# TimZaman/dotaclient

Measured on NVIDIA H100. Metric: optimizer_steps_per_sec, higher is better.
Workload: dtype f32

## Files before the change

### dotaclient_b200/csrc/gemm_tf32x3.cu

```cuda
#include "dc_common.cuh"
#include "unit_basic.cuh"

namespace {

constexpr int BM = 128, BN = 128, BK = 32;
constexpr int kStages = 2;
constexpr int kTileBytes = BM * BK * 4;
constexpr int kStageBytes = 4 * kTileBytes;
constexpr int kProducerThreads = 128;
constexpr int kProducerGroups = kStages;
constexpr int kConsumerWarp0 = 4 * kProducerGroups;
constexpr int kConsumerThreads = 256;
constexpr int kThreads = kConsumerWarp0 * 32 + kConsumerThreads;
constexpr int kLdS = BN + 8;
constexpr int kDIn = kUnitFeatures;
constexpr size_t kOffStaging = (size_t)kStages * kStageBytes;
constexpr size_t kOffBars = kOffStaging + (size_t)BM * kLdS * 4;
constexpr size_t kSmemBytes = kOffBars + 128 + 1024 ;

#define DC_ACC8(b) "+f"(d[b]), "+f"(d[b + 1]), "+f"(d[b + 2]), "+f"(d[b + 3]), "+f"(d[b + 4]), "+f"(d[b + 5]), "+f"(d[b + 6]), "+f"(d[b + 7])
__device__ __forceinline__ void wgmma_m64n128k8(float (&d)[64], uint64_t desc_a, uint64_t desc_b) {
    asm volatile(
        "{\n\t.reg .pred p;\n\tsetp.ne.b32 p, %66, 0;\n\t"
        "wgmma.mma_async.sync.aligned.m64n128k8.f32.tf32.tf32 "
// ... 130 lines not shown
            const float4 a4 = dl != nullptr ? __ldg(reinterpret_cast<const float4 *>(att + nn * 128 + k0) + c) : zero4;
            const float gl = dl != nullptr ? __ldg(dl + nn * ld_dl) : 0.f;
            raw.v[i] = ok ? make_float4(fmaf(gl, a4.x, d.x), fmaf(gl, a4.y, d.y), fmaf(gl, a4.z, d.z), fmaf(gl, a4.w, d.w)) : zero4;
        }
    } else {
        constexpr int kTileToks = (BM - BM % NU) / NU;
#pragma unroll
        for (int k = 0; k < DembRaw<NU>::kP; ++k) {
            const int p = t + kProducerThreads * k;
            const int c = p & 7, tokl = NU == 16 ? p >> 4 : p >> 3;
            const int u0 = NU == 16 ? ((p >> 3) & 1) * 8 : 0;
            const bool active = tokl < kTileToks;
            const int n = tok0 + tokl;
            raw.ok[k] = active && n < n_tok;
            const size_t nn = (size_t)min(n, n_tok - 1);
            float4 d = (active && dx != nullptr) ? __ldg(reinterpret_cast<const float4 *>(dx + nn * ld_dx + k0) + c) : zero4;
            const float4 d2 = (active && dx2 != nullptr) ? __ldg(reinterpret_cast<const float4 *>(dx2 + nn * ld_dx + k0) + c) : zero4;
            if constexpr (NU == 16) {
                raw.d2[k] = d2;
            } else {
                d.x += d2.x; d.y += d2.y; d.z += d2.z; d.w += d2.w;
            }
            raw.d[k] = d;
            raw.am[k] = (active && dx != nullptr) ? __ldg(reinterpret_cast<const uint32_t *>(argmax + nn * 128 + k0) + c) : 0u;
            raw.a[k] = (active && dl != nullptr) ? __ldg(reinterpret_cast<const float4 *>(att + nn * 128 + k0) + c) : zero4;
#pragma unroll
            for (int j = 0; j < DembRaw<NU>::kU; ++j) raw.g[k][j] = (active && dl != nullptr) ? __ldg(dl + nn * ld_dl + u0 + j) : 0.f;
        }
    }
}

__device__ __forceinline__ void store_hi_lo(unsigned char *dst_hi, unsigned char *dst_lo, int off, float4 o) {
    float4 hi, lo;
    hi.x = dc_tf32_rna(o.x); hi.y = dc_tf32_rna(o.y); hi.z = dc_tf32_rna(o.z); hi.w = dc_tf32_rna(o.w);
    lo.x = o.x - hi.x; lo.y = o.y - hi.y; lo.z = o.z - hi.z; lo.w = o.w - hi.w;
    *reinterpret_cast<float4 *>(dst_hi + off) = hi;
    *reinterpret_cast<float4 *>(dst_lo + off) = lo;
}

template <int NU>
__device__ __forceinline__ void demb_store(const DembRaw<NU> &raw, unsigned char *dst_hi, unsigned char *dst_lo, int t) {
    if constexpr (NU == 1) {
        tile_store_k(raw.v, dst_hi, dst_lo, t);
    } else {
        constexpr int kTileRows = BM - BM % NU, kTileToks = kTileRows / NU;
        const float4 zero4 = make_float4(0.f, 0.f, 0.f, 0.f);
#pragma unroll
        for (int k = 0; k < DembRaw<NU>::kP; ++k) {
            const int p = t + kProducerThreads * k;
            const int c = p & 7, tokl = NU == 16 ? p >> 4 : p >> 3;
            const int u0 = NU == 16 ? ((p >> 3) & 1) * 8 : 0;
            if (tokl < kTileToks) {
                float4 d = raw.d[k];
                if constexpr (NU == 16) { d.x += raw.d2[k].x; d.y += raw.d2[k].y; d.z += raw.d2[k].z; d.w += raw.d2[k].w; }
                const float4 a = raw.a[k];
                const uint32_t am = raw.am[k];
#pragma unroll
                for (int j = 0; j < DembRaw<NU>::kU; ++j) {
                    const int u = u0 + j, r = tokl * NU + u;
                    const float gl = raw.g[k][j];
                    float4 o;
                    o.x = fmaf(gl, a.x, (int)(am & 0xffu) == u ? d.x : 0.f);
                    o.y = fmaf(gl, a.y, (int)((am >> 8) & 0xffu) == u ? d.y : 0.f);
                    o.z = fmaf(gl, a.z, (int)((am >> 16) & 0xffu) == u ? d.z : 0.f);
                    o.w = fmaf(gl, a.w, (int)(am >> 24) == u ? d.w : 0.f);
                    store_hi_lo(dst_hi, dst_lo, r * 128 + ((c ^ (r & 7)) << 4), raw.ok[k] ? o : zero4);
                }
            }
        }
        if constexpr (kTileRows < BM) {
            if (t < (BM - kTileRows) * 8) {
                const int r = kTileRows + (t >> 3), c = t & 7;
                store_hi_lo(dst_hi, dst_lo, r * 128 + ((c ^ (r & 7)) << 4), zero4);
            }
        }
    }
}

__device__ __forceinline__ void store_row_k(const float (&v)[32], unsigned char *dst_hi, unsigned char *dst_lo, int row) {
#pragma unroll
    for (int c = 0; c < 8; ++c) {
        const int off = row * 128 + ((c ^ (row & 7)) << 4);
        float4 hi, lo;
        hi.x = dc_tf32_rna(v[4 * c]); hi.y = dc_tf32_rna(v[4 * c + 1]); hi.z = dc_tf32_rna(v[4 * c + 2]); hi.w = dc_tf32_rna(v[4 * c + 3]);
        lo.x = v[4 * c] - hi.x; lo.y = v[4 * c + 1] - hi.y; lo.z = v[4 * c + 2] - hi.z; lo.w = v[4 * c + 3] - hi.w;
        *reinterpret_cast<float4 *>(dst_hi + off) = hi;
        *reinterpret_cast<float4 *>(dst_lo + off) = lo;
    }
}

__global__ void __launch_bounds__(kThreads, 1) gemm_tf32x3_kernel(const float *__restrict__ A, int lda,
                                                                  const float *__restrict__ B, int ldb,
                                                                  const float *__restrict__ bias, float *__restrict__ C,
                                                                  int ldc, int M, int N, int K, int relu, int ksplit,
                                                                  long long c_split_stride) {
    constexpr int kTileRows = BM;
    extern __shared__ unsigned char smem_raw[];
    unsigned char *tiles = smem_base(smem_raw);
    float *S = reinterpret_cast<float *>(tiles + kOffStaging);
    uint64_t *full = reinterpret_cast<uint64_t *>(tiles + kOffBars), *empty = full + kStages;

    const int warp = threadIdx.x >> 5, lane = threadIdx.x & 31;
    const int m_blocks = (M + kTileRows - 1) / kTileRows, n_blocks = (N + BN - 1) / BN, k_chunks = K / BK / ksplit;
    const int tiles_mn = m_blocks * n_blocks, tiles_total = tiles_mn * ksplit;
    init_ring(full);

    if (warp < kConsumerWarp0) {
        const int t = threadIdx.x & (kProducerThreads - 1), g = warp >> 2;
        uint32_t c = 0;
        for (int tile = blockIdx.x; tile < tiles_total; tile += gridDim.x) {
            const int tmn = tile % tiles_mn, kc0 = (tile / tiles_mn) * k_chunks;
            const int m0 = (tmn / n_blocks) * kTileRows, n0 = (tmn % n_blocks) * BN;
            for (int kc = 0; kc < k_chunks; ++kc, ++c) {
                if ((int)(c % kProducerGroups) != g) continue;
                float4 va[8], vb[8];
                tile_load_k(A, lda, m0, M, (kc0 + kc) * BK, t, va);
                tile_load_k(B, ldb, n0, N, (kc0 + kc) * BK, t, vb);
                produce(full, empty, c, lane, [&](int s) {
                    unsigned char *st = tiles + (size_t)s * kStageBytes;
                    tile_store_k(va, st, st + kTileBytes, t);
                    tile_store_k(vb, st + 2 * kTileBytes, st + 3 * kTileBytes, t);
                });
            }
        }
    } else {
        const int ct = threadIdx.x - kConsumerWarp0 * 32, wg = ct >> 7, cw = ct >> 5;
        float d[64];
        uint32_t c = 0;
        for (int tile = blockIdx.x; tile < tiles_total; tile += gridDim.x) {
            const int tmn = tile % tiles_mn, sp = tile / tiles_mn;
            const int m0 = (tmn / n_blocks) * kTileRows, n0 = (tmn % n_blocks) * BN;
            consume(d, tiles, full, empty, c, k_chunks, wg, lane);
            consumer_sync();
            stage_acc(d, S, ct);
            consumer_sync();
            const bool lane_in = n0 + 4 * lane < N;
            const bool has_bias = bias != nullptr && sp == 0 && lane_in;
            const float4 b4 = has_bias ? __ldg(reinterpret_cast<const float4 *>(bias + n0) + lane) : make_float4(0.f, 0.f, 0.f, 0.f);
            float *cbase = C + (size_t)sp * (size_t)c_split_stride + n0 + 4 * lane;
            for (int r = cw; lane_in && r < BM && m0 + r < M; r += kConsumerThreads / 32) {
                float4 v = *reinterpret_cast<const float4 *>(S + r * kLdS + 4 * lane);
                if (has_bias) { v.x += b4.x; v.y += b4.y; v.z += b4.z; v.w += b4.w; }
                if (relu) { v.x = fmaxf(v.x, 0.f); v.y = fmaxf(v.y, 0.f); v.z = fmaxf(v.z, 0.f); v.w = fmaxf(v.w, 0.f); }
                *reinterpret_cast<float4 *>(cbase + (size_t)(m0 + r) * ldc) = v;
            }
        }
    }
}

constexpr int kWsRows = 64;
constexpr int kWsStages = 8;
constexpr int kWsChunkBytes = kWsRows * BK * 4;
constexpr int kWsThreads = kConsumerThreads + 128;
constexpr int kWsLdS = 40;
constexpr size_t kWsOffRing = (size_t)4 * 2 * kTileBytes;
constexpr size_t kWsOffStaging = kWsOffRing + (size_t)kWsStages * kWsChunkBytes;
constexpr size_t kWsOffBars = kWsOffStaging + (size_t)(kConsumerThreads / 32) * 16 * kWsLdS * 4;
constexpr size_t kWsSmemBytes = kWsOffBars + 2 * kWsStages * 8 + 1024 ;
constexpr size_t kWsOffUnits = kWsOffBars + 2 * kWsStages * 8;
constexpr size_t kWsGenSmemBytes = kWsOffUnits + (size_t)4 * kWsRows * kDIn * 4 + 1024 ;
static_assert(kWsSmemBytes <= 227 * 1024 && kWsGenSmemBytes <= 227 * 1024, "weight-stationary GEMM exceeds the shared-memory opt-in");
static_assert(kWsOffUnits % 16 == 0, "unit rows are staged with 16-byte stores");

struct GenA {
    const float *units, *w_b, *b_b;
    float *basic_out;
    uint32_t *mask_out;
};

__device__ __forceinline__ void cp_async16(uint32_t dst, const void *src, uint32_t src_bytes) {
    asm volatile("cp.async.cg.shared.global [%0], [%1], 16, %2;" ::"r"(dst), "l"(src), "r"(src_bytes) : "memory");
}
__device__ __forceinline__ void cp_async_arrive(uint64_t *bar) {
    asm volatile("cp.async.mbarrier.arrive.noinc.shared::cta.b64 [%0];" ::"r"(dc_smem_u32(bar)) : "memory");
}

#define DC_ACC8(b) "+f"(d[b]), "+f"(d[b + 1]), "+f"(d[b + 2]), "+f"(d[b + 3]), "+f"(d[b + 4]), "+f"(d[b + 5]), "+f"(d[b + 6]), "+f"(d[b + 7])
__device__ __forceinline__ void wgmma_m64n128k8_rs(float (&d)[64], uint32_t a0, uint32_t a1, uint32_t a2, uint32_t a3, uint64_t desc_b) {
    asm volatile(
        "{\n\t.reg .pred p;\n\tsetp.ne.b32 p, %69, 0;\n\t"
        "wgmma.mma_async.sync.aligned.m64n128k8.f32.tf32.tf32 "
        "{%0, %1, %2, %3, %4, %5, %6, %7, %8, %9, %10, %11, %12, %13, %14, %15, "
        "%16, %17, %18, %19, %20, %21, %22, %23, %24, %25, %26, %27, %28, %29, %30, %31, "
        "%32, %33, %34, %35, %36, %37, %38, %39, %40, %41, %42, %43, %44, %45, %46, %47, "
        "%48, %49, %50, %51, %52, %53, %54, %55, %56, %57, %58, %59, %60, %61, %62, %63}, "
        "{%64, %65, %66, %67}, %68, p, 1, 1;\n\t}\n"
        : DC_ACC8(0), DC_ACC8(8), DC_ACC8(16), DC_ACC8(24), DC_ACC8(32), DC_ACC8(40), DC_ACC8(48), DC_ACC8(56)
        : "r"(a0), "r"(a1), "r"(a2), "r"(a3), "l"(desc_b), "r"(1));
}
#undef DC_ACC8

__device__ __forceinline__ void ws_fetch(float (&v)[16], const float *chunk, int rlo, int rhi, bool hi_ok, int q) {
#pragma unroll
    for (int ks = 0; ks < BK / 8; ++ks) {
#pragma unroll
        for (int h = 0; h < 2; ++h) {
            const int j = 2 * ks + h;
            v[4 * ks + 2 * h] = chunk[rlo * BK + ((j ^ (rlo & 7)) << 2) + q];
            v[4 * ks + 2 * h + 1] = hi_ok ? chunk[rhi * BK + ((j ^ (rhi & 7)) << 2) + q] : 0.f;
        }
    }
}

template <int NU, bool kGenA>
__global__ void __launch_bounds__(kWsThreads, 1) gemm_ws_kernel(const float *__restrict__ A, int lda,
                                                                const float *__restrict__ B, int ldb,
                                                                const float *__restrict__ bias, float *__restrict__ C,
                                                                int ldc, int M, int N, int K, int relu,
                                                                float *__restrict__ C_copy, uint8_t *__restrict__ argmax, GenA gen) {
    constexpr int kWarpRows = NU == 5 ? 15 : 16;
    constexpr int kTileRows = 4 * kWarpRows;
    extern __shared__ unsigned char smem_raw[];
    unsigned char *sm = smem_base(smem_raw);
    unsigned char *ring = sm + kWsOffRing;
    uint64_t *full = reinterpret_cast<uint64_t *>(sm + kWsOffBars), *empty = full + kWsStages;

    const int warp = threadIdx.x >> 5, lane = threadIdx.x & 31;
    const int n_blocks = (N + BN - 1) / BN, m_blocks = (M + kTileRows - 1) / kTileRows, k_chunks = K / BK;
    const int n0 = (blockIdx.x % n_blocks) * BN, mb0 = blockIdx.x / n_blocks, mstride = gridDim.x / n_blocks;
    if (threadIdx.x == 0) {
        for (int s = 0; s < kWsStages; ++s) { dc_mbar_init(&full[s], kGenA ? 1 : 128); dc_mbar_init(&empty[s], 4); }
        asm volatile("fence.mbarrier_init.release.cluster;" ::: "memory");
    }
    __syncthreads();

    if constexpr (kGenA) if (warp >= kConsumerThreads / 32) {
        const int kc = warp - kConsumerThreads / 32, ch = lane & 7, r0 = lane >> 3;
        const int j0 = kc * BK + 4 * ch;
        float wb[4][kDIn], bb[4];
#pragma unroll
        for (int e = 0; e < 4; ++e) {
            bb[e] = __ldg(gen.b_b + j0 + e);
#pragma unroll
            for (int k = 0; k < kDIn; ++k) wb[e][k] = __ldg(gen.w_b + (j0 + e) * kDIn + k);
        }
        float4 *su = reinterpret_cast<float4 *>(sm + kWsOffUnits) + kc * (kWsRows * kDIn / 4);
        const float4 *units4 = reinterpret_cast<const float4 *>(gen.units);
        constexpr int kU4 = kWsRows * kDIn / 4 / 32;
        float4 nxt[kU4];
        auto fetch = [&](int mb) {
            const bool live = mb < m_blocks;
            const int m0 = live ? mb * kTileRows : 0;
#pragma unroll
            for (int i = 0; i < kU4; ++i) {
                const int idx = lane + 32 * i, r = idx / 3;
                nxt[i] = (live && r < kTileRows && m0 + r < M) ? __ldg(units4 + (size_t)m0 * 3 + idx) : make_float4(0.f, 0.f, 0.f, 0.f);
            }
        };
        fetch(mb0);
        uint32_t c = kc;
        for (int mb = mb0; mb < m_blocks; mb += mstride, c += 4) {
            const int m0 = mb * kTileRows;
            __syncwarp();
#pragma unroll
            for (int i = 0; i < kU4; ++i) su[lane + 32 * i] = nxt[i];
            __syncwarp();
            fetch(mb + mstride);
            const int s = c % kWsStages;
            dc_mbar_wait(&empty[s], ((c / kWsStages) & 1) ^ 1);
            unsigned char *chunk = ring + (size_t)s * kWsChunkBytes;
#pragma unroll 4
            for (int i = 0; i < kWsRows / 4; ++i) {
                const int r = r0 + 4 * i;
                const bool ok = r < kTileRows && m0 + r < M;
                const float4 u0 = su[3 * r], u1 = su[3 * r + 1], u2 = su[3 * r + 2];
                const float u[kDIn] = {u0.x, u0.y, u0.z, u0.w, u1.x, u1.y, u1.z, u1.w, u2.x, u2.y, u2.z, u2.w};
                float4 v = make_float4(dc_unit_basic(u, wb[0], bb[0]), dc_unit_basic(u, wb[1], bb[1]), dc_unit_basic(u, wb[2], bb[2]),
                                       dc_unit_basic(u, wb[3], bb[3]));
                if (!ok) v = make_float4(0.f, 0.f, 0.f, 0.f);
                *reinterpret_cast<float4 *>(chunk + r * 128 + ((ch ^ (r & 7)) << 4)) = v;
                if (gen.basic_out != nullptr && ok) *reinterpret_cast<float4 *>(gen.basic_out + (size_t)(m0 + r) * BN + j0) = v;
            }
            __syncwarp();
            if (lane == 0) dc_mbar_arrive(&full[s]);
        }
        return;
    }
    if constexpr (!kGenA) if (warp >= kConsumerThreads / 32) {
        const int p = threadIdx.x - kConsumerThreads, ch = p & 7;
        uint32_t c = 0;
        for (int mb = mb0; mb < m_blocks; mb += mstride) {
            const int m0 = mb * kTileRows;
            for (int kc = 0; kc < k_chunks; ++kc, ++c) {
                const int s = c % kWsStages;
                dc_mbar_wait(&empty[s], ((c / kWsStages) & 1) ^ 1);
                const uint32_t dst = dc_smem_u32(ring + (size_t)s * kWsChunkBytes);
#pragma unroll
                for (int i = 0; i < kWsRows / 16; ++i) {
                    const int r = (p >> 3) + 16 * i;
                    const bool ok = r < kTileRows && m0 + r < M;
                    const float *src = A + (ok ? (size_t)(m0 + r) * lda : 0) + kc * BK + 4 * ch;
                    cp_async16(dst + r * 128 + ((ch ^ (r & 7)) << 4), src, ok ? 16u : 0u);
                }
                cp_async_arrive(&full[s]);
            }
        }
        asm volatile("cp.async.wait_all;" ::: "memory");
        return;
    }

    const int wg = warp >> 2, w4 = warp & 3, t = threadIdx.x & 127, q = lane & 3, g8 = lane >> 2;
    {
        for (int kc = wg; kc < k_chunks; kc += 2) {
            float4 vb[8];
            tile_load_k(B, ldb, n0, N, kc * BK, t, vb);
            tile_store_k(vb, sm + (size_t)kc * 2 * kTileBytes, sm + (size_t)kc * 2 * kTileBytes + kTileBytes, t);
        }
        asm volatile("fence.proxy.async.shared::cta;" ::: "memory");
        consumer_sync();
    }
    const uint32_t w_base = dc_smem_u32(sm);
    const int rlo = kWarpRows * w4 + g8, rhi = rlo + 8;
    const bool hi_ok = NU != 5 || g8 < 7;
    float *Sw = reinterpret_cast<float *>(sm + kWsOffStaging) + warp * 16 * kWsLdS;
    float d[64];
    uint32_t c = 0;
    int i = 0;
    for (int mb = mb0; mb < m_blocks; mb += mstride, ++i, c += k_chunks) {
        if ((i & 1) != wg) continue;
        const int m0 = mb * kTileRows;
        uint32_t mask_lo = 0, mask_hi = 0;
#pragma unroll
        for (int j = 0; j < 64; ++j) d[j] = 0.f;
        float v[16];
        uint32_t ahi[16], alo[16];
        {
            const int s = c % kWsStages;
            dc_mbar_wait(&full[s], (c / kWsStages) & 1);
            ws_fetch(v, reinterpret_cast<const float *>(ring + (size_t)s * kWsChunkBytes), rlo, rhi, hi_ok, q);
        }
        for (int kc = 0; kc < k_chunks; ++kc) {
#pragma unroll
            for (int j = 0; j < 16; ++j) {
                const float h = dc_tf32_rna(v[j]);
                ahi[j] = __float_as_uint(h);
                alo[j] = __float_as_uint(v[j] - h);
            }
            __syncwarp();
            if (lane == 0) dc_mbar_arrive(&empty[(c + kc) % kWsStages]);
#pragma unroll
            for (int j = 0; j < 64; ++j) dc_reg_fence(d[j]);
            dc_wgmma_fence();
            const uint64_t b_hi = dc_wgmma_desc(w_base + kc * 2 * kTileBytes), b_lo = dc_wgmma_desc(w_base + kc * 2 * kTileBytes + kTileBytes);
#pragma unroll
            for (int ks = 0; ks < BK / 8; ++ks) {
                const uint64_t adv = (uint64_t)(ks * 2);
                wgmma_m64n128k8_rs(d, alo[4 * ks], alo[4 * ks + 1], alo[4 * ks + 2], alo[4 * ks + 3], b_hi + adv);
                wgmma_m64n128k8_rs(d, ahi[4 * ks], ahi[4 * ks + 1], ahi[4 * ks + 2], ahi[4 * ks + 3], b_lo + adv);
                wgmma_m64n128k8_rs(d, ahi[4 * ks], ahi[4 * ks + 1], ahi[4 * ks + 2], ahi[4 * ks + 3], b_hi + adv);
            }
            dc_wgmma_commit();
            if (kGenA && gen.mask_out != nullptr) {
                uint32_t lo = 0, hi = 0;
#pragma unroll
                for (int ks = 0; ks < BK / 8; ++ks) {
#pragma unroll
                    for (int h = 0; h < 2; ++h) {
                        lo |= v[4 * ks + 2 * h] > 0.f ? 1u << (2 * ks + h) : 0u;
                        hi |= v[4 * ks + 2 * h + 1] > 0.f ? 1u << (2 * ks + h) : 0u;
                    }
                }
                mask_lo |= lo << (8 * kc);
                mask_hi |= hi << (8 * kc);
            }
            if (kc + 1 < k_chunks) {
                const uint32_t cn = c + kc + 1;
                const int s = cn % kWsStages;
                dc_mbar_wait(&full[s], (cn / kWsStages) & 1);
                ws_fetch(v, reinterpret_cast<const float *>(ring + (size_t)s * kWsChunkBytes), rlo, rhi, hi_ok, q);
            }
            dc_wgmma_wait0();
#pragma unroll
            for (int j = 0; j < 16; ++j) asm volatile("" : "+r"(ahi[j]), "+r"(alo[j])::"memory");
#pragma unroll
            for (int j = 0; j < 64; ++j) dc_reg_fence(d[j]);
        }
        if (kGenA && gen.mask_out != nullptr) {
            if (m0 + rlo < M) gen.mask_out[(size_t)(m0 + rlo) * 4 + q] = mask_lo;
            if (hi_ok && m0 + rhi < M) gen.mask_out[(size_t)(m0 + rhi) * 4 + q] = mask_hi;
        }

        if constexpr (NU == 0) {
            const int row_lo = m0 + rlo, row_hi = m0 + rhi;
            float *c_lo = row_lo < M ? C + (size_t)row_lo * ldc : nullptr, *c_hi = row_hi < M ? C + (size_t)row_hi * ldc : nullptr;
#pragma unroll
            for (int g = 0; g < BN / 8; ++g) {
                const int col = n0 + 8 * g + 2 * q;
                if (col >= N) break;
                const float2 b2 = bias != nullptr ? __ldg(reinterpret_cast<const float2 *>(bias + col)) : make_float2(0.f, 0.f);
                float2 lo = make_float2(d[4 * g], d[4 * g + 1]), hi = make_float2(d[4 * g + 2], d[4 * g + 3]);
                if (bias != nullptr) { lo.x += b2.x; lo.y += b2.y; hi.x += b2.x; hi.y += b2.y; }
                if (relu) { lo.x = fmaxf(lo.x, 0.f); lo.y = fmaxf(lo.y, 0.f); hi.x = fmaxf(hi.x, 0.f); hi.y = fmaxf(hi.y, 0.f); }
                if (c_lo) *reinterpret_cast<float2 *>(c_lo + col) = lo;
                if (c_hi) *reinterpret_cast<float2 *>(c_hi + col) = hi;
            }
        } else {
            constexpr int kToks = kWarpRows / NU;
            const int tok0 = m0 / NU + kToks * w4, n_tok = M / NU;
#pragma unroll
            for (int b = 0; b < BN / 32; ++b) {
#pragma unroll
                for (int g = 0; g < 4; ++g) {
                    const int j = 4 * (4 * b + g);
                    *reinterpret_cast<float2 *>(Sw + g8 * kWsLdS + 8 * g + 2 * q) = make_float2(d[j], d[j + 1]);
                    *reinterpret_cast<float2 *>(Sw + (g8 + 8) * kWsLdS + 8 * g + 2 * q) = make_float2(d[j + 2], d[j + 3]);
                }
                __syncwarp();
                const int col = 32 * b + lane;
                const float bias_f = __ldg(bias + col);
#pragma unroll
                for (int tk = 0; tk < kToks; ++tk) {
                    const int tok = tok0 + tk;
                    if (tok >= n_tok) break;
                    const float *p = Sw + tk * NU * kWsLdS + lane;
                    float best = p[0];
                    int best_u = 0;
#pragma unroll
                    for (int u = 1; u < NU; ++u) {
                        const float x = p[u * kWsLdS];
                        if (x > best) { best = x; best_u = u; }
                    }
                    const float o = best + bias_f;
                    C[(size_t)tok * ldc + col] = o;
                    if (C_copy) C_copy[(size_t)tok * ldc + col] = o;
                    argmax[(size_t)tok * BN + col] = (uint8_t)best_u;
                }
                __syncwarp();
            }
        }
    }
}

constexpr int kDgN = 16;
constexpr int kDgUTile = kDgN * BK * 4;
constexpr int kDgStageBytes = 2 * kTileBytes;
constexpr size_t kDgOffRing = (size_t)(BN / BK) * 2 * kTileBytes;
constexpr size_t kDgOffU = kDgOffRing + (size_t)kStages * kDgStageBytes;
constexpr int kDgFlush = 32;
constexpr int kDgMaskLd = BM + 8;
constexpr size_t kDgOffMask = kDgOffU + (size_t)2 * (BM / BK) * kDgUTile;
constexpr size_t kDgOffWb = kDgOffMask + (size_t)4 * kDgMaskLd * 4;
constexpr size_t kDgOffBars = kDgOffWb + (size_t)BN * (kDIn + 1) * 4;
constexpr size_t kDgSmemBytes = kDgOffBars + 2 * (kStages + 1) * 8 + 1024 ;
static_assert(kDgSmemBytes <= 227 * 1024, "unit data-gradient kernel exceeds the shared-memory opt-in");
static_assert(kDgOffU % 1024 == 0 && kDgUTile % 1024 == 0, "the swizzled U tiles need 1024-byte alignment");

__device__ __forceinline__ void wgmma_wait1() { asm volatile("wgmma.wait_group.sync.aligned 1;" ::: "memory"); }

__device__ __forceinline__ void wgmma_m64n16k8_rs(float (&d)[8], const uint32_t (&a)[4], uint64_t desc_b) {
    asm volatile(
        "{\n\t.reg .pred p;\n\tsetp.ne.b32 p, %13, 0;\n\t"
        "wgmma.mma_async.sync.aligned.m64n16k8.f32.tf32.tf32 {%0, %1, %2, %3, %4, %5, %6, %7}, {%8, %9, %10, %11}, %12, p, 1, 1;\n\t}\n"
        : "+f"(d[0]), "+f"(d[1]), "+f"(d[2]), "+f"(d[3]), "+f"(d[4]), "+f"(d[5]), "+f"(d[6]), "+f"(d[7])
        : "r"(a[0]), "r"(a[1]), "r"(a[2]), "r"(a[3]), "l"(desc_b), "r"(1));
}

struct DgAux {
    float4 u[3];
    uint32_t m[4];
    bool ok;
};

template <bool kMask>
__device__ __forceinline__ void aux_fetch(DgAux &x, const float *__restrict__ units, const uint32_t *__restrict__ mask, int m0,
                                          int rows_valid, int t) {
    const float4 zero4 = make_float4(0.f, 0.f, 0.f, 0.f);
    x.ok = t < rows_valid;
    const size_t row = (size_t)(m0 + (x.ok ? t : 0));
#pragma unroll
    for (int i = 0; i < 3; ++i) x.u[i] = x.ok ? __ldg(reinterpret_cast<const float4 *>(units) + row * 3 + i) : zero4;
    if constexpr (kMask) {
        const uint4 w = x.ok ? __ldg(reinterpret_cast<const uint4 *>(mask) + row) : make_uint4(0u, 0u, 0u, 0u);
        x.m[0] = w.x; x.m[1] = w.y; x.m[2] = w.z; x.m[3] = w.w;
    }
}

__device__ __forceinline__ void aux_recompute_mask(DgAux &x, const float *sw, const float *sb) {
    const float u[kDIn] = {x.u[0].x, x.u[0].y, x.u[0].z, x.u[0].w, x.u[1].x, x.u[1].y, x.u[1].z, x.u[1].w, x.u[2].x, x.u[2].y, x.u[2].z, x.u[2].w};
#pragma unroll
    for (int w = 0; w < 4; ++w) {
        uint32_t bits = 0;
#pragma unroll 4
        for (int i = 0; i < 32; ++i) {
            const int j = 4 * i + w;
            const float4 *wr4 = reinterpret_cast<const float4 *>(sw + j * kDIn);
            const float4 w0 = wr4[0], w1 = wr4[1], w2 = wr4[2];
            const float wr[kDIn] = {w0.x, w0.y, w0.z, w0.w, w1.x, w1.y, w1.z, w1.w, w2.x, w2.y, w2.z, w2.w};
            bits |= (dc_unit_basic(u, wr, sb[j]) > 0.f ? 1u : 0u) << i;
        }
        x.m[w] = x.ok ? bits : 0u;
    }
}

__device__ __forceinline__ void aux_store(const DgAux &x, unsigned char *sm_u, uint32_t *sm_mask, int t) {
    const int k = 8 * (t >> 3) + ((t & 7) >> 1) + 4 * (t & 1), kk = k & 31;
    unsigned char *base = sm_u + (k >> 5) * kDgUTile + (kk & 3) * 4;
    const float v[kDgN] = {x.u[0].x, x.u[0].y, x.u[0].z, x.u[0].w, x.u[1].x, x.u[1].y, x.u[1].z, x.u[1].w,
                           x.u[2].x, x.u[2].y, x.u[2].z, x.u[2].w, x.ok ? 1.f : 0.f, 0.f, 0.f, 0.f};
#pragma unroll
    for (int n = 0; n < kDgN; ++n) {
        const float hi = dc_tf32_rna(v[n]);
        const int off = n * 128 + (((kk >> 2) ^ (n & 7)) << 4);
        *reinterpret_cast<float *>(base + off) = hi;
        *reinterpret_cast<float *>(base + (BM / BK) * kDgUTile + off) = v[n] - hi;
    }
#pragma unroll
    for (int w = 0; w < 4; ++w) sm_mask[w * kDgMaskLd + t] = x.m[w];
}

template <int NU, bool kMask>
__global__ void __launch_bounds__(kThreads, 1) unit_dgrad_kernel(const float *__restrict__ dx, const float *__restrict__ dx2, int ld_dx,
                                                                 const uint8_t *__restrict__ argmax,
                                                                 const float *__restrict__ dl, int ld_dl,
                                                                 const float *__restrict__ att,
                                                                 const float *__restrict__ Wt, const float *__restrict__ units,
                                                                 const uint32_t *__restrict__ mask,
                                                                 const float *__restrict__ w_b, const float *__restrict__ b_b,
                                                                 int n_tok, float *__restrict__ partial) {
    constexpr int kTileRows = BM - BM % NU, kTileToks = kTileRows / NU;
    constexpr int k_chunks = BN / BK;
    extern __shared__ unsigned char smem_raw[];
    unsigned char *sm = smem_base(smem_raw);
    unsigned char *ring = sm + kDgOffRing, *sm_u = sm + kDgOffU;
    uint32_t *sm_mask = reinterpret_cast<uint32_t *>(sm + kDgOffMask);
    float *sm_wb = reinterpret_cast<float *>(sm + kDgOffWb), *sm_bb = sm_wb + BN * kDIn;
    uint64_t *full = reinterpret_cast<uint64_t *>(sm + kDgOffBars), *empty = full + kStages;
    uint64_t *ufull = empty + kStages, *uempty = ufull + 1;

    const int warp = threadIdx.x >> 5, lane = threadIdx.x & 31;
    const int M = n_tok * NU;
    const int m_blocks = (M + kTileRows - 1) / kTileRows;
    if constexpr (!kMask) {
        for (int i = threadIdx.x; i < BN * kDIn; i += kThreads) sm_wb[i] = __ldg(w_b + i);
        for (int i = threadIdx.x; i < BN; i += kThreads) sm_bb[i] = __ldg(b_b + i);
    }
    if (threadIdx.x == 0) {
        dc_mbar_init(ufull, 4);
        dc_mbar_init(uempty, kConsumerThreads / 32);
    }
    init_ring(full);

    if (warp < kConsumerWarp0) {
        const int t = threadIdx.x & (kProducerThreads - 1), g = warp >> 2;
        uint32_t c = 0;
        int it = 0;
        for (int mb = blockIdx.x; mb < m_blocks; mb += gridDim.x, ++it) {
            const int tok0 = mb * kTileToks, m0 = mb * kTileRows;
            for (int kc = 0; kc < k_chunks; ++kc, ++c) {
                if ((int)(c % kProducerGroups) != g) continue;
                DembRaw<NU> raw;
                DgAux aux;
                demb_fetch<NU>(raw, dx, dx2, ld_dx, argmax, dl, ld_dl, att, tok0, n_tok, kc * BK, t);
                if (kc == 0) aux_fetch<kMask>(aux, units, mask, m0, min(kTileRows, M - m0), t);
                produce(full, empty, c, lane, [&](int s) { demb_store<NU>(raw, ring + (size_t)s * kDgStageBytes, ring + (size_t)s * kDgStageBytes + kTileBytes, t); });
                if (kc == 0) {
                    if constexpr (!kMask) aux_recompute_mask(aux, sm_wb, sm_bb);
                    dc_mbar_wait(uempty, (it & 1) ^ 1);
                    aux_store(aux, sm_u, sm_mask, t);
                    asm volatile("fence.proxy.async.shared::cta;" ::: "memory");
                    __syncwarp();
                    if (lane == 0) dc_mbar_arrive(ufull);
                }
            }
        }
    } else {
        const int ct = threadIdx.x - kConsumerWarp0 * 32, wg = ct >> 7, w4 = (ct >> 5) & 3, t = ct & 127, q4 = lane & 3;
        for (int kc = wg; kc < k_chunks; kc += 2) {
            float4 vb[8];
            tile_load_k(Wt, BN, 0, BN, kc * BK, t, vb);
            tile_store_k(vb, sm + (size_t)kc * 2 * kTileBytes, sm + (size_t)kc * 2 * kTileBytes + kTileBytes, t);
        }
        asm volatile("fence.proxy.async.shared::cta;" ::: "memory");
        consumer_sync();
        const uint32_t w_base = dc_smem_u32(sm) + wg * (64 * 128), ring_base = dc_smem_u32(ring), u_base = dc_smem_u32(sm_u);
        const int j_lo = 64 * wg + 16 * w4 + (lane >> 2);
        const uint32_t bit_lo = 1u << (j_lo >> 2), bit_hi = bit_lo << 2;
        const uint32_t *mrow = sm_mask + (j_lo & 3) * kDgMaskLd + 2 * q4;
        float acc[8];
#pragma unroll
        for (int i = 0; i < 8; ++i) acc[i] = 0.f;
        float *pp = partial + (size_t)blockIdx.x * BN * (kDIn + 1);
        const auto flush = [&](bool add) {
#pragma unroll
            for (int i = 0; i < 8; ++i) {
                const int j = j_lo + 8 * ((i >> 1) & 1), n = 8 * (i >> 2) + 2 * q4 + (i & 1);
                if (n <= kDIn) {
                    if (add) atomicAdd(pp + j * (kDIn + 1) + n, acc[i]);
                    else pp[j * (kDIn + 1) + n] = acc[i];
                }
                acc[i] = 0.f;
            }
#pragma unroll
            for (int i = 0; i < 8; ++i) dc_reg_fence(acc[i]);
        };
        float d[64];
        uint32_t c = 0;
        int it = 0;
        for (int mb = blockIdx.x; mb < m_blocks; mb += gridDim.x, ++it) {
#pragma unroll
            for (int i = 0; i < 64; ++i) d[i] = 0.f;
// ... 155 lines not shown
            __syncwarp();
            if (lane == 0) dc_mbar_arrive(&full[s]);
        }
        colsum_s[g * 128 + t] = cs;
        asm volatile("cp.async.wait_all;" ::: "memory");
    } else {
        const int ct = threadIdx.x - kConsumerWarp0 * 32, wg = ct >> 7, w4 = (ct >> 5) & 3, q = lane & 3;
        const int rlo = 64 * wg + 16 * w4 + (lane >> 2);
        float d[64];
#pragma unroll
        for (int i = 0; i < 64; ++i) d[i] = 0.f;
        uint32_t ahi[2][4] = {}, alo[2][4] = {};
#pragma unroll
        for (int i = 0; i < 64; ++i) dc_reg_fence(d[i]);
        float *pt = part_w + ((size_t)split * tiles_mn + tile) * BM * BN + ct * 4;
        const auto flush = [&](bool add) {
            dc_wgmma_wait0();
#pragma unroll
            for (int k = 0; k < 64; ++k) dc_reg_fence(d[k]);
            if (add) {
#pragma unroll
                for (int m = 0; m < 16; ++m)
                    asm volatile("red.global.add.v4.f32 [%0], {%1, %2, %3, %4};" ::"l"(pt + m * kConsumerThreads * 4), "f"(d[4 * m]),
                                 "f"(d[4 * m + 1]), "f"(d[4 * m + 2]), "f"(d[4 * m + 3]) : "memory");
            } else {
#pragma unroll
                for (int m = 0; m < 16; ++m)
                    *reinterpret_cast<float4 *>(pt + m * kConsumerThreads * 4) = make_float4(d[4 * m], d[4 * m + 1], d[4 * m + 2], d[4 * m + 3]);
            }
#pragma unroll
            for (int k = 0; k < 64; ++k) d[k] = 0.f;
#pragma unroll
            for (int k = 0; k < 64; ++k) dc_reg_fence(d[k]);
        };
        int j = 0;
        do {
            const int j_end = min(my_chunks, j + kWgFlush);
            for (; j < j_end; ++j) {
                const int s = j % kWgStages;
                dc_mbar_wait(&full[s], (j / kWgStages) & 1);
                const uint32_t st = dc_smem_u32(ring + (size_t)s * kWgStageBytes);
                const uint32_t xk = st + 2 * kTileBytes + (q * kWgLdX + rlo) * 4;
                float v[16];
#pragma unroll
                for (int ks = 0; ks < BK / 8; ++ks) {
                    const uint32_t x8 = xk + 8 * ks * kWgLdX * 4;
                    v[4 * ks] = lds_f32(x8);
                    v[4 * ks + 1] = lds_f32(x8 + 8 * 4);
                    v[4 * ks + 2] = lds_f32(x8 + 4 * kWgLdX * 4);
                    v[4 * ks + 3] = lds_f32(x8 + (4 * kWgLdX + 8) * 4);
                }
                const uint64_t b_hi = dc_wgmma_desc(st), b_lo = dc_wgmma_desc(st + kTileBytes);
#pragma unroll
                for (int ks = 0; ks < BK / 8; ++ks) {
                    const int b = ks & 1;
#pragma unroll
                    for (int e = 0; e < 4; ++e) {
                        const float h = dc_tf32_rna(v[4 * ks + e]);
                        ahi[b][e] = __float_as_uint(h);
                        alo[b][e] = __float_as_uint(v[4 * ks + e] - h);
                    }
                    dc_wgmma_fence();
                    const uint64_t adv = (uint64_t)(ks * 2);
                    wgmma_m64n128k8_rs(d, ahi[b][0], ahi[b][1], ahi[b][2], ahi[b][3], b_lo + adv);
                    wgmma_m64n128k8_rs(d, alo[b][0], alo[b][1], alo[b][2], alo[b][3], b_hi + adv);
                    wgmma_m64n128k8_rs(d, ahi[b][0], ahi[b][1], ahi[b][2], ahi[b][3], b_hi + adv);
                    dc_wgmma_commit();
                    wgmma_wait1();
#pragma unroll
                    for (int e = 0; e < 4; ++e) asm volatile("" : "+r"(ahi[b ^ 1][e]), "+r"(alo[b ^ 1][e])::"memory");
                    if (ks == 0 && j > 0) {
                        __syncwarp();
                        if (lane == 0) dc_mbar_arrive(&empty[(j - 1) % kWgStages]);
                    }
                }
            }
            flush(j > kWgFlush);
        } while (j < my_chunks);
    }
    __syncthreads();
    if (part_b != nullptr && n0 == 0 && threadIdx.x < 128 && m0 + (int)threadIdx.x < No)
        part_b[(size_t)split * No + m0 + threadIdx.x] = colsum_s[threadIdx.x] + colsum_s[128 + threadIdx.x];
}

constexpr int kRedRows = 8;
__global__ void __launch_bounds__(32 * kRedRows) wgrad_reduce_kernel(const float *__restrict__ part_w, const float *__restrict__ part_b,
                                                                     int nsplit, int No, int Ni, float *__restrict__ dW, int ldw,
                                                                     float *__restrict__ db, int accumulate) {
    __shared__ float4 sh[kRedRows][32];
    const int x = threadIdx.x & 31, y = threadIdx.x >> 5;
    const int n_blocks = (Ni + BN - 1) / BN, tiles_mn = ((No + BM - 1) / BM) * n_blocks;
    const int total4 = tiles_mn * (BM * BN / 4), bias4 = db != nullptr ? No / 4 : 0;
    const int idx = blockIdx.x * 32 + x;
    const float *src = nullptr;
    size_t stride = 0;
    if (idx < total4) {
        src = part_w + (size_t)idx * 4;
        stride = (size_t)tiles_mn * BM * BN;
    } else if (idx < total4 + bias4) {
        src = part_b + (size_t)(idx - total4) * 4;
        stride = (size_t)No;
    }
    float4 acc = make_float4(0.f, 0.f, 0.f, 0.f);
    if (src != nullptr) {
#pragma unroll 4
        for (int s = y; s < nsplit; s += kRedRows) {
            const float4 v = __ldg(reinterpret_cast<const float4 *>(src + (size_t)s * stride));
            acc.x += v.x; acc.y += v.y; acc.z += v.z; acc.w += v.w;
        }
    }
    sh[y][x] = acc;
    __syncthreads();
    if (y == 0 && src != nullptr) {
        if (idx < total4) {
            const int tile = idx / (BM * BN / 4), r = idx % (BM * BN / 4), m = r / kConsumerThreads, ct = r % kConsumerThreads;
            const int o = (tile / n_blocks) * BM + 8 * m + 2 * (ct & 3);
            const int i = (tile % n_blocks) * BN + 64 * (ct >> 7) + 16 * ((ct >> 5) & 3) + ((ct & 31) >> 2);
            float *p[4];
            float v[4];
#pragma unroll
            for (int e = 0; e < 4; ++e) {
                const int oe = o + (e & 1), ie = i + 8 * (e >> 1);
                p[e] = oe < No && ie < Ni ? dW + (size_t)oe * ldw + ie : nullptr;
                v[e] = accumulate && p[e] != nullptr ? *p[e] : 0.f;
            }
#pragma unroll
            for (int r = 0; r < kRedRows; ++r) { v[0] += sh[r][x].x; v[1] += sh[r][x].y; v[2] += sh[r][x].z; v[3] += sh[r][x].w; }
#pragma unroll
            for (int e = 0; e < 4; ++e)
                if (p[e] != nullptr) *p[e] = v[e];
        } else {
            float *dst = db + (size_t)(idx - total4) * 4;
            float4 t = accumulate ? *reinterpret_cast<const float4 *>(dst) : make_float4(0.f, 0.f, 0.f, 0.f);
#pragma unroll
            for (int r = 0; r < kRedRows; ++r) { t.x += sh[r][x].x; t.y += sh[r][x].y; t.z += sh[r][x].z; t.w += sh[r][x].w; }
            *reinterpret_cast<float4 *>(dst) = t;
        }
    }
}

}

extern "C" int dc_gemm_tf32x3_supported(int64_t M, int N, int K) { return M > 0 && N > 0 && K > 0 && N % 32 == 0 && K % BK == 0; }

template <int NU, bool kGenA = false>
static int launch_ws(const float *A, int lda, const float *B, int ldb, const float *bias, float *C, int ldc, int M, int N,
                     int K, int relu, float *C_copy, uint8_t *argmax, cudaStream_t st, GenA gen = GenA{}) {
    const int tile_rows = NU == 5 ? 60 : kWsRows;
    const int n_blocks = (N + BN - 1) / BN, m_blocks = (M + tile_rows - 1) / tile_rows;
    int per_block = dc_sm_count() / n_blocks;
    if (per_block < 1) per_block = 1;
    if (per_block > m_blocks) per_block = m_blocks;
    const size_t smem = kGenA ? kWsGenSmemBytes : kWsSmemBytes;
    DC_CUDA(cudaFuncSetAttribute(gemm_ws_kernel<NU, kGenA>, cudaFuncAttributeMaxDynamicSharedMemorySize, (int)smem));
    gemm_ws_kernel<NU, kGenA><<<n_blocks * per_block, kWsThreads, smem, st>>>(A, lda, B, ldb, bias, C, ldc, M, N, K, relu, C_copy,
                                                                             argmax, gen);
    DC_LAUNCH_OK();
    return DC_OK;
}

extern "C" int dc_gemm_tf32x3(const float *A, int lda, const float *B, int ldb, const float *bias, float *C, int ldc,
                              int64_t M, int N, int K, int relu, dc_stream_t stream) {
    DC_REQUIRE(A && B && C, DC_EINVAL, "dc_gemm_tf32x3: null pointer");
    DC_REQUIRE(dc_gemm_tf32x3_supported(M, N, K) && M < (1ll << 31) - BM, DC_EUNSUPPORTED,
               "dc_gemm_tf32x3: need N %% 32 == 0 and K %% 32 == 0 (M=%lld N=%d K=%d)", (long long)M, N, K);
    DC_REQUIRE(lda >= K && ldb >= K && ldc >= N && lda % 4 == 0 && ldb % 4 == 0 && ldc % 4 == 0, DC_EINVAL,
               "dc_gemm_tf32x3: leading dimensions must be >= extent and multiples of 4 floats");
    DC_REQUIRE(((uintptr_t)A & 15) == 0 && ((uintptr_t)B & 15) == 0 && ((uintptr_t)C & 15) == 0 && (!bias || ((uintptr_t)bias & 15) == 0),
               DC_EINVAL, "dc_gemm_tf32x3: pointers must be 16-byte aligned");
    if (K <= 4 * BK) return launch_ws<0>(A, lda, B, ldb, bias, C, ldc, (int)M, N, K, relu, nullptr, nullptr, dc_cu_stream(stream));
    const int tiles = (int)((M + BM - 1) / BM) * ((N + BN - 1) / BN);
    DC_CUDA(cudaFuncSetAttribute(gemm_tf32x3_kernel, cudaFuncAttributeMaxDynamicSharedMemorySize, (int)kSmemBytes));
    const int grid = tiles < dc_sm_count() ? tiles : dc_sm_count();
    gemm_tf32x3_kernel<<<grid, kThreads, kSmemBytes, dc_cu_stream(stream)>>>(A, lda, B, ldb, bias, C, ldc, (int)M, N, K, relu, 1, 0);
    DC_LAUNCH_OK();
    return DC_OK;
}

int dc_gemm_tf32x3_splitk(const float *A, int lda, const float *B, int ldb, float *part, int64_t M, int N, int K, int ksplit,
                          bool first_call, cudaStream_t st) {
    DC_REQUIRE(A && B && part && ksplit >= 1 && N % BN == 0 && K % (BK * ksplit) == 0 && M > 0, DC_EINVAL,
               "dc_gemm_tf32x3_splitk: bad arguments (M=%lld N=%d K=%d ksplit=%d)", (long long)M, N, K, ksplit);
    if (first_call)
        DC_CUDA(cudaFuncSetAttribute(gemm_tf32x3_kernel, cudaFuncAttributeMaxDynamicSharedMemorySize, (int)kSmemBytes));
    const int tiles = (int)((M + BM - 1) / BM) * (N / BN) * ksplit;
    const int grid = tiles < dc_sm_count() ? tiles : dc_sm_count();
    gemm_tf32x3_kernel<<<grid, kThreads, kSmemBytes, st>>>(A, lda, B, ldb, nullptr, part, N, (int)M, N, K, 0, ksplit, (long long)M * N);
    DC_LAUNCH_OK();
    return DC_OK;
}

static int wgrad_tiles(int No, int Ni) { return ((No + BM - 1) / BM) * ((Ni + BN - 1) / BN); }

static int wgrad_splits(int No, int Ni) {
    const int tiles_mn = wgrad_tiles(No, Ni);
    const int n = dc_sm_count() / tiles_mn;
    return n < 1 ? 1 : n;
}

extern "C" size_t dc_gemm_wgrad_workspace_bytes(int No, int Ni) {
    if (No <= 0 || Ni <= 0 || No % 32 || Ni % 32) return 0;
    const int nsplit = wgrad_splits(No, Ni);
    return ((size_t)nsplit * wgrad_tiles(No, Ni) * BM * BN + (size_t)nsplit * No) * sizeof(float);
}

extern "C" int dc_gemm_wgrad_tf32x3(const float *dY, int ldy, const float *X, int ldx, int64_t T, int No, int Ni, float *dW,
                                    int ldw, float *db, int accumulate, void *workspace, dc_stream_t stream) {
    DC_REQUIRE(dY && X && dW && workspace, DC_EINVAL, "dc_gemm_wgrad_tf32x3: null pointer");
    DC_REQUIRE(T > 0 && T < (1ll << 31) - BK && No > 0 && Ni > 0 && No % 32 == 0 && Ni % 32 == 0, DC_EUNSUPPORTED,
               "dc_gemm_wgrad_tf32x3: need No %% 32 == 0 and Ni %% 32 == 0 (T=%lld No=%d Ni=%d)", (long long)T, No, Ni);
    DC_REQUIRE(ldy >= No && ldx >= Ni && ldw >= Ni && ldy % 4 == 0 && ldx % 4 == 0 && ldw % 4 == 0, DC_EINVAL,
               "dc_gemm_wgrad_tf32x3: bad leading dimension");
    DC_REQUIRE(((uintptr_t)dY & 15) == 0 && ((uintptr_t)X & 15) == 0 && ((uintptr_t)dW & 15) == 0 && ((uintptr_t)workspace & 15) == 0 &&
                   ((uintptr_t)db & 15) == 0,
               DC_EINVAL, "dc_gemm_wgrad_tf32x3: pointers must be 16-byte aligned");
    const int tiles_mn = wgrad_tiles(No, Ni), nsplit = wgrad_splits(No, Ni);
    float *part_w = reinterpret_cast<float *>(workspace);
    float *part_b = db ? part_w + (size_t)nsplit * tiles_mn * BM * BN : nullptr;
    cudaStream_t st = dc_cu_stream(stream);
    DC_CUDA(cudaFuncSetAttribute(gemm_wgrad_kernel<0>, cudaFuncAttributeMaxDynamicSharedMemorySize, (int)kWgSmemBytes));
    gemm_wgrad_kernel<0><<<tiles_mn * nsplit, kThreads, kWgSmemBytes, st>>>(dY, ldy, nullptr, nullptr, X, ldx, (int)T, No, Ni,
                                                                                      nsplit, part_w, part_b);
    DC_LAUNCH_OK();
    const int total4 = tiles_mn * (BM * BN / 4) + (db ? No / 4 : 0);
    wgrad_reduce_kernel<<<(total4 + 31) / 32, 32 * kRedRows, 0, st>>>(part_w, part_b, nsplit, No, Ni, dW, ldw, db, accumulate);
    DC_LAUNCH_OK();
    return DC_OK;
}

extern "C" int dc_gemm_unit_max(const float *basic, const float *w, const float *bias, float *xmax, float *xmax_copy, int ld_x,
                                uint8_t *argmax, int64_t n_tokens, int n_units, dc_stream_t stream) {
    DC_REQUIRE(basic && w && bias && xmax && argmax && n_tokens > 0, DC_EINVAL, "dc_gemm_unit_max: null pointer / empty input");
    DC_REQUIRE(n_units == 5 || n_units == 16, DC_EUNSUPPORTED, "dc_gemm_unit_max: n_units=%d (5 or 16; 1-unit groups are plain GEMMs)", n_units);
    DC_REQUIRE(ld_x >= BN && n_tokens * n_units < (1ll << 31) - BM, DC_EINVAL, "dc_gemm_unit_max: bad ld_x / size");
    DC_REQUIRE(((uintptr_t)basic & 15) == 0 && ((uintptr_t)w & 15) == 0, DC_EINVAL, "dc_gemm_unit_max: pointers must be 16-byte aligned");
    const int M = (int)(n_tokens * n_units);
    cudaStream_t st = dc_cu_stream(stream);
    if (n_units == 5) return launch_ws<5>(basic, BN, w, BN, bias, xmax, ld_x, M, BN, BN, 0, xmax_copy, argmax, st);
    return launch_ws<16>(basic, BN, w, BN, bias, xmax, ld_x, M, BN, BN, 0, xmax_copy, argmax, st);
}

extern "C" int dc_unit_embed_fwd_mask(const float *units, const float *w_b, const float *b_b, float *basic_out, uint32_t *mask_out,
                                      const float *w, const float *bias, float *xmax, float *xmax_copy, int ld_x, uint8_t *argmax,
                                      int64_t n_tokens, int n_units, dc_stream_t stream) {
    DC_REQUIRE(units && w_b && b_b && w && bias && xmax && n_tokens > 0, DC_EINVAL, "dc_unit_embed_fwd: null pointer / empty input");
    DC_REQUIRE(n_units == 1 || n_units == 5 || n_units == 16, DC_EUNSUPPORTED, "dc_unit_embed_fwd: n_units=%d (1, 5 or 16)", n_units);
    DC_REQUIRE(n_units == 1 ? (argmax == nullptr && xmax_copy == nullptr) : argmax != nullptr, DC_EINVAL,
               "dc_unit_embed_fwd: the arg-max (and the copy) go with the max-pool of n_units 5 and 16 only");
    DC_REQUIRE(ld_x >= BN && ld_x % 4 == 0 && n_tokens * n_units < (1ll << 31) - BM, DC_EINVAL, "dc_unit_embed_fwd: bad ld_x / size");
    DC_REQUIRE(((uintptr_t)units & 15) == 0 && ((uintptr_t)basic_out & 15) == 0 && ((uintptr_t)w & 15) == 0 && ((uintptr_t)bias & 15) == 0 &&
                   ((uintptr_t)xmax & 15) == 0 && ((uintptr_t)xmax_copy & 15) == 0 && ((uintptr_t)mask_out & 15) == 0,
               DC_EINVAL, "dc_unit_embed_fwd: units, basic_out, mask_out, w, bias, xmax, xmax_copy must be 16-byte aligned");
    const int M = (int)(n_tokens * n_units);
    const GenA gen{units, w_b, b_b, basic_out, mask_out};
    cudaStream_t st = dc_cu_stream(stream);
    if (n_units == 1) return launch_ws<0, true>(nullptr, BN, w, BN, bias, xmax, ld_x, M, BN, BN, 0, nullptr, nullptr, st, gen);
    if (n_units == 5) return launch_ws<5, true>(nullptr, BN, w, BN, bias, xmax, ld_x, M, BN, BN, 0, xmax_copy, argmax, st, gen);
    return launch_ws<16, true>(nullptr, BN, w, BN, bias, xmax, ld_x, M, BN, BN, 0, xmax_copy, argmax, st, gen);
}

extern "C" int dc_unit_embed_fwd(const float *units, const float *w_b, const float *b_b, float *basic_out, const float *w, const float *bias,
                                 float *xmax, float *xmax_copy, int ld_x, uint8_t *argmax, int64_t n_tokens, int n_units,
                                 dc_stream_t stream) {
    return dc_unit_embed_fwd_mask(units, w_b, b_b, basic_out, nullptr, w, bias, xmax, xmax_copy, ld_x, argmax, n_tokens, n_units, stream);
}

extern "C" int dc_unit_dgrad_fused_mask(const float *d_xmax, const float *d_xmax2, int ld_dx, const uint8_t *argmax, const float *dlogits,
                                        int ld_dl, const float *att, const float *w_t, const float *units, const uint32_t *mask,
                                        const float *w_b, const float *b_b, int64_t n_tokens, int n_units, float *dw_b, float *db_b,
                                        int accumulate, void *workspace, dc_stream_t stream) {
    DC_REQUIRE(w_t && units && w_b && b_b && dw_b && db_b && workspace && n_tokens > 0, DC_EINVAL, "dc_unit_dgrad_fused: null pointer / empty input");
    DC_REQUIRE(n_units == 1 || n_units == 5 || n_units == 16, DC_EUNSUPPORTED, "dc_unit_dgrad_fused: n_units=%d (1, 5 or 16)", n_units);
    DC_REQUIRE((d_xmax == nullptr && d_xmax2 == nullptr) || (d_xmax != nullptr && ld_dx >= BN && ld_dx % 4 == 0), DC_EINVAL,
               "dc_unit_dgrad_fused: bad d_xmax / ld_dx");
    DC_REQUIRE(d_xmax == nullptr || n_units == 1 || argmax != nullptr, DC_EINVAL, "dc_unit_dgrad_fused: routing needs the arg-max");
    DC_REQUIRE((dlogits == nullptr) == (att == nullptr) && (dlogits == nullptr || ld_dl >= n_units), DC_EINVAL,
               "dc_unit_dgrad_fused: dlogits and att come together");
    DC_REQUIRE(n_tokens * n_units < (1ll << 31) - BM, DC_EINVAL, "dc_unit_dgrad_fused: too many rows");
    DC_REQUIRE(((uintptr_t)d_xmax & 15) == 0 && ((uintptr_t)d_xmax2 & 15) == 0 && ((uintptr_t)argmax & 3) == 0 && ((uintptr_t)att & 15) == 0 &&
                   ((uintptr_t)w_t & 15) == 0 && ((uintptr_t)units & 15) == 0 && ((uintptr_t)mask & 15) == 0 && ((uintptr_t)workspace & 15) == 0,
               DC_EINVAL, "dc_unit_dgrad_fused: d_xmax, att, w_t, units, mask must be 16-byte aligned (arg-max 4-byte)");
    const int n_tok = (int)n_tokens;
    const int tile_rows = BM - BM % n_units;
    int grid = (int)((n_tokens * n_units + tile_rows - 1) / tile_rows);
    if (grid > dc_sm_count()) grid = dc_sm_count();
    float *partial = reinterpret_cast<float *>(workspace);
    cudaStream_t st = dc_cu_stream(stream);
#define DC_LAUNCH_DGRAD(NU, MASK)                                                                                                    \
    do {                                                                                                                              \
        DC_CUDA(cudaFuncSetAttribute(unit_dgrad_kernel<NU, MASK>, cudaFuncAttributeMaxDynamicSharedMemorySize, (int)kDgSmemBytes)); \
        unit_dgrad_kernel<NU, MASK><<<grid, kThreads, kDgSmemBytes, st>>>(d_xmax, d_xmax2, ld_dx, argmax, dlogits, ld_dl, att, w_t,  \
                                                                          units, mask, w_b, b_b, n_tok, partial);                     \
    } while (0)
    if (mask != nullptr) {
        if (n_units == 1) DC_LAUNCH_DGRAD(1, true);
        else if (n_units == 5) DC_LAUNCH_DGRAD(5, true);
        else DC_LAUNCH_DGRAD(16, true);
    } else {
        if (n_units == 1) DC_LAUNCH_DGRAD(1, false);
        else if (n_units == 5) DC_LAUNCH_DGRAD(5, false);
        else DC_LAUNCH_DGRAD(16, false);
    }
#undef DC_LAUNCH_DGRAD
    DC_LAUNCH_OK();
    return dc_unit_basic_reduce(partial, grid, dw_b, db_b, accumulate, st);
}

extern "C" int dc_unit_dgrad_fused(const float *d_xmax, const float *d_xmax2, int ld_dx, const uint8_t *argmax, const float *dlogits,
                                   int ld_dl, const float *att, const float *w_t, const float *units, const float *w_b,
// ... 33 lines not shown
```

Baseline: 75.37.

## Double-buffer A fragments and keep one wgmma group in flight in weight-stationary GEMM

The weight-stationary GEMM consumer loop now double-buffers the split hi/lo TF32 A fragments and waits with wait_group 1 instead of 0. The next chunk's split can then overlap the previous chunk's asynchronous wgmma. K-chunk count becomes a template parameter so the loop fully unrolls, and setmaxnreg rebalances registers from producer to consumer warps in the non-generating variant. The cost is more template instantiations and higher register pressure in the consumers, with some risk of spills.

New measurement: 76.71 (median of 6 runs). No clear change (+1.8%).

```diff
diff --git a/dotaclient_b200/csrc/gemm_tf32x3.cu b/dotaclient_b200/csrc/gemm_tf32x3.cu
--- a/dotaclient_b200/csrc/gemm_tf32x3.cu
+++ b/dotaclient_b200/csrc/gemm_tf32x3.cu
@@ -306,6 +306,7 @@
 constexpr int kWsStages = 8;
 constexpr int kWsChunkBytes = kWsRows * BK * 4;
 constexpr int kWsThreads = kConsumerThreads + 128;
+constexpr int kWsConsumerRegs = 232, kWsProducerRegs = 40;
 constexpr int kWsLdS = 40;
 constexpr size_t kWsOffRing = (size_t)4 * 2 * kTileBytes;
 constexpr size_t kWsOffStaging = kWsOffRing + (size_t)kWsStages * kWsChunkBytes;
@@ -328,6 +329,7 @@
 __device__ __forceinline__ void cp_async_arrive(uint64_t *bar) {
     asm volatile("cp.async.mbarrier.arrive.noinc.shared::cta.b64 [%0];" ::"r"(dc_smem_u32(bar)) : "memory");
 }
+__device__ __forceinline__ void wgmma_wait1() { asm volatile("wgmma.wait_group.sync.aligned 1;" ::: "memory"); }
 
 #define DC_ACC8(b) "+f"(d[b]), "+f"(d[b + 1]), "+f"(d[b + 2]), "+f"(d[b + 3]), "+f"(d[b + 4]), "+f"(d[b + 5]), "+f"(d[b + 6]), "+f"(d[b + 7])
 __device__ __forceinline__ void wgmma_m64n128k8_rs(float (&d)[64], uint32_t a0, uint32_t a1, uint32_t a2, uint32_t a3, uint64_t desc_b) {
@@ -356,12 +358,13 @@
     }
 }
 
-template <int NU, bool kGenA>
+template <int NU, bool kGenA, int KC>
 __global__ void __launch_bounds__(kWsThreads, 1) gemm_ws_kernel(const float *__restrict__ A, int lda,
                                                                 const float *__restrict__ B, int ldb,
                                                                 const float *__restrict__ bias, float *__restrict__ C,
-                                                                int ldc, int M, int N, int K, int relu,
+                                                                int ldc, int M, int N, int relu,
                                                                 float *__restrict__ C_copy, uint8_t *__restrict__ argmax, GenA gen) {
+    static_assert(KC >= 1 && KC <= 4 && (!kGenA || KC == 4), "K <= 128; the basic layer has 128 channels");
     constexpr int kWarpRows = NU == 5 ? 15 : 16;
     constexpr int kTileRows = 4 * kWarpRows;
     extern __shared__ unsigned char smem_raw[];
@@ -370,13 +373,19 @@
     uint64_t *full = reinterpret_cast<uint64_t *>(sm + kWsOffBars), *empty = full + kWsStages;
 
     const int warp = threadIdx.x >> 5, lane = threadIdx.x & 31;
-    const int n_blocks = (N + BN - 1) / BN, m_blocks = (M + kTileRows - 1) / kTileRows, k_chunks = K / BK;
+    const int n_blocks = (N + BN - 1) / BN, m_blocks = (M + kTileRows - 1) / kTileRows;
+    constexpr int k_chunks = KC;
     const int n0 = (blockIdx.x % n_blocks) * BN, mb0 = blockIdx.x / n_blocks, mstride = gridDim.x / n_blocks;
     if (threadIdx.x == 0) {
         for (int s = 0; s < kWsStages; ++s) { dc_mbar_init(&full[s], kGenA ? 1 : 128); dc_mbar_init(&empty[s], 4); }
         asm volatile("fence.mbarrier_init.release.cluster;" ::: "memory");
     }
     __syncthreads();
+
+    if constexpr (!kGenA) {
+        if (warp >= kConsumerThreads / 32) asm volatile("setmaxnreg.dec.sync.aligned.u32 %0;" ::"n"(kWsProducerRegs));
+        else asm volatile("setmaxnreg.inc.sync.aligned.u32 %0;" ::"n"(kWsConsumerRegs));
+    }
 
     if constexpr (kGenA) if (warp >= kConsumerThreads / 32) {
         const int kc = warp - kConsumerThreads / 32, ch = lane & 7, r0 = lane >> 3;
@@ -468,27 +477,33 @@
     const bool hi_ok = NU != 5 || g8 < 7;
     float *Sw = reinterpret_cast<float *>(sm + kWsOffStaging) + warp * 16 * kWsLdS;
     float d[64];
+    uint32_t ahi[2][16], alo[2][16];
+#pragma unroll
+    for (int j = 0; j < 16; ++j) ahi[0][j] = alo[0][j] = ahi[1][j] = alo[1][j] = 0u;
     uint32_t c = 0;
     int i = 0;
     for (int mb = mb0; mb < m_blocks; mb += mstride, ++i, c += k_chunks) {
         if ((i & 1) != wg) continue;
         const int m0 = mb * kTileRows;
         uint32_t mask_lo = 0, mask_hi = 0;
+        float v[16];
+        const auto fetch = [&](int kc) {
+            const uint32_t cn = c + kc;
+            const int s = cn % kWsStages;
+            dc_mbar_wait(&full[s], (cn / kWsStages) & 1);
+            ws_fetch(v, reinterpret_cast<const float *>(ring + (size_t)s * kWsChunkBytes), rlo, rhi, hi_ok, q);
+        };
 #pragma unroll
         for (int j = 0; j < 64; ++j) d[j] = 0.f;
-        float v[16];
-        uint32_t ahi[16], alo[16];
-        {
-            const int s = c % kWsStages;
-            dc_mbar_wait(&full[s], (c / kWsStages) & 1);
-            ws_fetch(v, reinterpret_cast<const float *>(ring + (size_t)s * kWsChunkBytes), rlo, rhi, hi_ok, q);
-        }
+        fetch(0);
+#pragma unroll(kGenA ? 1 : KC)
         for (int kc = 0; kc < k_chunks; ++kc) {
+            const int b = kGenA ? 0 : kc & 1;
 #pragma unroll
             for (int j = 0; j < 16; ++j) {
                 const float h = dc_tf32_rna(v[j]);
-                ahi[j] = __float_as_uint(h);
-                alo[j] = __float_as_uint(v[j] - h);
+                ahi[b][j] = __float_as_uint(h);
+                alo[b][j] = __float_as_uint(v[j] - h);
             }
             __syncwarp();
             if (lane == 0) dc_mbar_arrive(&empty[(c + kc) % kWsStages]);
@@ -499,9 +514,9 @@
 #pragma unroll
             for (int ks = 0; ks < BK / 8; ++ks) {
                 const uint64_t adv = (uint64_t)(ks * 2);
-                wgmma_m64n128k8_rs(d, alo[4 * ks], alo[4 * ks + 1], alo[4 * ks + 2], alo[4 * ks + 3], b_hi + adv);
-                wgmma_m64n128k8_rs(d, ahi[4 * ks], ahi[4 * ks + 1], ahi[4 * ks + 2], ahi[4 * ks + 3], b_lo + adv);
-                wgmma_m64n128k8_rs(d, ahi[4 * ks], ahi[4 * ks + 1], ahi[4 * ks + 2], ahi[4 * ks + 3], b_hi + adv);
+                wgmma_m64n128k8_rs(d, alo[b][4 * ks], alo[b][4 * ks + 1], alo[b][4 * ks + 2], alo[b][4 * ks + 3], b_hi + adv);
+                wgmma_m64n128k8_rs(d, ahi[b][4 * ks], ahi[b][4 * ks + 1], ahi[b][4 * ks + 2], ahi[b][4 * ks + 3], b_lo + adv);
+                wgmma_m64n128k8_rs(d, ahi[b][4 * ks], ahi[b][4 * ks + 1], ahi[b][4 * ks + 2], ahi[b][4 * ks + 3], b_hi + adv);
             }
             dc_wgmma_commit();
             if (kGenA && gen.mask_out != nullptr) {
@@ -517,18 +532,17 @@
                 mask_lo |= lo << (8 * kc);
                 mask_hi |= hi << (8 * kc);
             }
-            if (kc + 1 < k_chunks) {
-                const uint32_t cn = c + kc + 1;
-                const int s = cn % kWsStages;
-                dc_mbar_wait(&full[s], (cn / kWsStages) & 1);
-                ws_fetch(v, reinterpret_cast<const float *>(ring + (size_t)s * kWsChunkBytes), rlo, rhi, hi_ok, q);
-            }
-            dc_wgmma_wait0();
-#pragma unroll
-            for (int j = 0; j < 16; ++j) asm volatile("" : "+r"(ahi[j]), "+r"(alo[j])::"memory");
-#pragma unroll
-            for (int j = 0; j < 64; ++j) dc_reg_fence(d[j]);
-        }
+            if (kc + 1 < k_chunks) fetch(kc + 1);
+            if constexpr (kGenA) dc_wgmma_wait0();
+            else wgmma_wait1();
+#pragma unroll
+            for (int j = 0; j < 16; ++j) asm volatile("" : "+r"(ahi[b ^ 1][j]), "+r"(alo[b ^ 1][j])::"memory");
+        }
+        dc_wgmma_wait0();
+#pragma unroll
+        for (int j = 0; j < 16; ++j) asm volatile("" : "+r"(ahi[0][j]), "+r"(alo[0][j]), "+r"(ahi[1][j]), "+r"(alo[1][j])::"memory");
+#pragma unroll
+        for (int j = 0; j < 64; ++j) dc_reg_fence(d[j]);
         if (kGenA && gen.mask_out != nullptr) {
             if (m0 + rlo < M) gen.mask_out[(size_t)(m0 + rlo) * 4 + q] = mask_lo;
             if (hi_ok && m0 + rhi < M) gen.mask_out[(size_t)(m0 + rhi) * 4 + q] = mask_hi;
@@ -598,8 +612,6 @@
 constexpr size_t kDgSmemBytes = kDgOffBars + 2 * (kStages + 1) * 8 + 1024 ;
 static_assert(kDgSmemBytes <= 227 * 1024, "unit data-gradient kernel exceeds the shared-memory opt-in");
 static_assert(kDgOffU % 1024 == 0 && kDgUTile % 1024 == 0, "the swizzled U tiles need 1024-byte alignment");
-
-__device__ __forceinline__ void wgmma_wait1() { asm volatile("wgmma.wait_group.sync.aligned 1;" ::: "memory"); }
 
 __device__ __forceinline__ void wgmma_m64n16k8_rs(float (&d)[8], const uint32_t (&a)[4], uint64_t desc_b) {
     asm volatile(
@@ -1061,9 +1073,23 @@
     if (per_block < 1) per_block = 1;
     if (per_block > m_blocks) per_block = m_blocks;
     const size_t smem = kGenA ? kWsGenSmemBytes : kWsSmemBytes;
-    DC_CUDA(cudaFuncSetAttribute(gemm_ws_kernel<NU, kGenA>, cudaFuncAttributeMaxDynamicSharedMemorySize, (int)smem));
-    gemm_ws_kernel<NU, kGenA><<<n_blocks * per_block, kWsThreads, smem, st>>>(A, lda, B, ldb, bias, C, ldc, M, N, K, relu, C_copy,
-                                                                             argmax, gen);
+#define DC_LAUNCH_WS(KC)                                                                                                        \
+    do {                                                                                                                         \
+        DC_CUDA(cudaFuncSetAttribute(gemm_ws_kernel<NU, kGenA, KC>, cudaFuncAttributeMaxDynamicSharedMemorySize, (int)smem));         \
+        gemm_ws_kernel<NU, kGenA, KC><<<n_blocks * per_block, kWsThreads, smem, st>>>(A, lda, B, ldb, bias, C, ldc, M, N, relu,          \
+                                                                                             C_copy, argmax, gen);               \
+    } while (0)
+    if constexpr (NU == 0 && !kGenA) {
+        switch (K / BK) {
+            case 1: DC_LAUNCH_WS(1); break;
+            case 2: DC_LAUNCH_WS(2); break;
+            case 3: DC_LAUNCH_WS(3); break;
+            default: DC_LAUNCH_WS(4); break;
+        }
+    } else {
+        DC_LAUNCH_WS(4);
+    }
+#undef DC_LAUNCH_WS
     DC_LAUNCH_OK();
     return DC_OK;
 }
```
